# jkulhanek/viewformer

Hardware: NVIDIA H100
Metric: novel views/sec (128x128, 9-ctx) (higher is better)
Workload: dtype f32 encoder (bit-exact codes) + bf16 transformer/decoder

## Files before the change

### include/vf_b200.h

```cpp
#ifndef VF_B200_H
#define VF_B200_H

#include <stdint.h>

#ifdef __cplusplus
extern "C" {
#endif

typedef void* vf_stream_t;

enum { VF_F32 = 0, VF_BF16 = 1, VF_F16X2 = 2  };
enum { VF_ACT_NONE = 0, VF_ACT_GELU_ERF = 1 };
enum { VF_BIAS_NONE = 0, VF_BIAS_N = 1, VF_BIAS_M = 2 };
enum { VF_OK = 0, VF_ERR_ARG = -1, VF_ERR_CUDA = -2, VF_ERR_UNSUPPORTED = -3 };

const char* vf_last_error(void);
int vf_version(void);
int vf_sizeof_simt_gemm(void);
int vf_sizeof_tc_gemm(void);
int vf_device_check(void);

int vf_u8_to_unit_f32(const uint8_t* in, float* out, int64_t rows, int64_t row_len, int64_t in_row_stride, vf_stream_t s);
int vf_unit_f32_to_u8(const float* in, uint8_t* out, int64_t n, vf_stream_t s);
int vf_nchw_to_nhwc_f32(const float* in, float* out, int N, int C, int H, int W, vf_stream_t s);
// ... 17 lines not shown
                 void* y, int y_dtype, vf_stream_t s);

typedef struct {
    const void* A; int a_dtype; int conv;
    int N, H, W, Cin;
    int OH, OW, KH, KW, stride, pad_t, pad_l, upsample2x;
    int64_t a_sm, a_sk;
    const void* B; int b_dtype; int64_t b_sk, b_sn;
    int M, Ncols, K;
    int batch1, batch2;
    int64_t a_sb1, a_sb2, b_sb1, b_sb2, c_sb1, c_sb2;
    float alpha; const float* bias; int bias_mode; int act;
    const float* residual;
    float* C_f32; void* C_bf16;
    int64_t ldc;
} vf_simt_gemm_t;
int vf_simt_gemm(const vf_simt_gemm_t* p, vf_stream_t s);

typedef struct {
    int conv;
    int ab_dtype;
    const void* A; const void* B;
    int M, Ncols, K; int batch1, batch2;
    int64_t lda, ldb;
    int64_t a_sb1, a_sb2, b_sb1, b_sb2;
    int N, H, W, Ctot, Cin, OH, OW, ntaps;
    int tap_dy[9], tap_dx[9], tap_coff[9];
    int causal_block, causal_skip_n;
    float alpha; const float* bias; int bias_mode; int act; const float* residual;
    float* C_f32; void* C_bf16; int64_t ldc, c_sb1, c_sb2;
    double* gn_sums; int gn_groups; int gn_rows_per_img;
    const float* norm_mean_rstd; const float* norm_gamma; const float* norm_beta; int norm_groups; int norm_swish;
    int64_t exact_lo_a, exact_lo_b;
} vf_tc_gemm_t;
int vf_tc_gemm(const vf_tc_gemm_t* p, vf_stream_t s);

int vf_attn_block_causal(const void* qk, const void* vt, int B, int S, int H, int d, int block, void* out, vf_stream_t s);
int vf_attn_block_causal_tail(const void* qk_bf16, const void* vt_bf16, int B, int S, int H, int d, int block, int first_query,
                              void* out_bf16, vf_stream_t s);
int vf_attn_block_causal_decode(const void* qk_bf16, const void* vt_bf16, int B, int S, int H, int d, int block, int first_query,
                                int skip_view, void* out_bf16, vf_stream_t s);
int vf_attn_block_multiend(const void* qk_bf16, const void* vt_bf16, int B, int S, int n_streams, int stream, int H, int d, int block,
                           void* out_bf16, vf_stream_t s);
int vf_attn_multiend_train(const void* qk_bf16, const void* vt_bf16, int B, int S, int n_streams, int stream, int H, int d, int block,
                           float rate, uint64_t seed, float* lse, float* out_f32, void* out_bf16, vf_stream_t s);
int vf_attn_multiend_bwd(const void* qk_bf16, const void* vt_bf16, const void* dout_bf16, const float* out, const float* lse, int B, int S,
                         int n_streams, int H, int d, int block, float rate, uint64_t seed, float* dvqk, vf_stream_t s);

int vf_conv_wgrad(const float* x, const float* dy, int N, int H, int W, int Cin, int OH, int OW, int Cout, int KH, int KW, int stride,
                  int pad_t, int pad_l, int upsample2x, int64_t so_k, int64_t so_n, float* dw, vf_stream_t s);
int vf_col_sums(const float* x, int64_t rows, int C, float* out, vf_stream_t s);
int vf_groupnorm_bwd(const float* x, const float* dout, const float* mean_rstd, const float* gamma, const float* beta, int N, int HW,
                     int C, int groups, int swish, const float* add, double* gsums, float* dgamma, float* dbeta, float* dx, void* dx_bf16,
                     vf_stream_t s);
int vf_softmax_bwd_rows(const float* P, const float* dP, int64_t rows, int cols, float* dS, vf_stream_t s);
int vf_l1_grad(const float* x, const float* y, int64_t n, float scale, float* dy, double* loss_sum, vf_stream_t s);
int vf_lincomb3(float a, const float* x, float b, const float* y, float c, const float* z, int64_t n, float* out, vf_stream_t s);
int vf_pad_transpose_split(const float* x_nhwc, int N, int H, int W, int C, int pitch, int copies, int64_t margin, int64_t L, void* out_f16,
                           vf_stream_t s);
int vf_sum_splits(const float* partial, int groups, int splits, int64_t n, int accumulate, float* out, vf_stream_t s);
typedef struct { const float* w_kn; void* fw_bf16; void* bw_bf16; int64_t cin, cout; } vf_conv_weights_bf16_t;
int vf_pad_transpose_bf16(const float* x_nhwc, int N, int H, int W, int C, int upsample2x, int pitch, int copies, int64_t margin, int64_t L,
                          const float* mean_rstd, const float* gamma, const float* beta, int groups, int swish, void* out_bf16, vf_stream_t s);
int vf_conv_weights_bf16(const vf_conv_weights_bf16_t* table, int n, vf_stream_t s);
int vf_sumpool2x2(const float* x, int N, int H, int W, int C, float* y, vf_stream_t s);
int vf_adam(float* p, const float* g, float* m, float* v, int64_t n, float lr, float beta1, float beta2, float eps, int step,
// ... 61 lines not shown
```

### viewformer_b200/_lib.py

```python
import ctypes as C
import os

import torch

HERE = os.path.dirname(os.path.abspath(__file__))
LIB_PATH = os.environ.get("VF_B200_LIB") or os.path.join(HERE, "libvf_b200.so")

F32, BF16, F16X2 = 0, 1, 2
ACT_NONE, ACT_GELU = 0, 1
BIAS_NONE, BIAS_N, BIAS_M = 0, 1, 2

EXPORTS = [
    "vf_last_error", "vf_version", "vf_sizeof_simt_gemm", "vf_sizeof_tc_gemm", "vf_device_check", "vf_u8_to_unit_f32", "vf_unit_f32_to_u8",
    "vf_nchw_to_nhwc_f32", "vf_nhwc_to_nchw_f32", "vf_groupnorm_stats", "vf_groupnorm_apply", "vf_layernorm",
    "vf_simt_gemm", "vf_tc_gemm", "vf_vq_lookup", "vf_gather_rows", "vf_vq_ema_stats", "vf_vq_ema_update", "vf_vq_commit_grad",
    "vf_vq_prepare_codebook", "vf_migt_embed", "vf_softmax_rows", "vf_argmax_rows", "vf_pose_postprocess",
    "vf_cameras_prepare", "vf_cameras_from_relative",
    "vf_conv3x3_small_cin", "vf_conv3x3_small_cout", "vf_groupnorm_finalize", "vf_split_f16x2", "vf_attn_block_causal", "vf_attn_block_causal_tail", "vf_attn_block_causal_decode", "vf_attn_block_multiend",
    "vf_vq_split3", "vf_vq_select", "vf_cross_entropy_rows", "vf_pose_loss_rows", "vf_row_mean",
    "vf_vq_prepare_codebook_f16", "vf_vq_lookup_fused", "vf_resize_u8", "vf_image_pair_sums", "vf_ssim_u8", "vf_ssim_u8_k",
    "vf_conv_wgrad", "vf_pad_transpose_split", "vf_pad_transpose_bf16", "vf_conv_weights_bf16", "vf_sum_splits", "vf_col_sums", "vf_groupnorm_bwd", "vf_softmax_bwd_rows", "vf_l1_grad", "vf_lincomb3", "vf_sumpool2x2", "vf_adam",
    "vf_layernorm_bwd", "vf_gelu_fwd", "vf_gelu_bwd", "vf_migt_embed_bwd", "vf_cross_entropy_grad", "vf_pose_loss_grad", "vf_adamw_keras", "vf_sumsq", "vf_dropout",
    "vf_attn_multiend_train", "vf_attn_multiend_bwd", "vf_to_bf16", "vf_dense_weights_bf16",
]
# ... 1 lines not shown

class SimtGemm(C.Structure):
    _fields_ = [
        ("A", C.c_void_p), ("a_dtype", C.c_int), ("conv", C.c_int),
        ("N", C.c_int), ("H", C.c_int), ("W", C.c_int), ("Cin", C.c_int),
        ("OH", C.c_int), ("OW", C.c_int), ("KH", C.c_int), ("KW", C.c_int), ("stride", C.c_int),
        ("pad_t", C.c_int), ("pad_l", C.c_int), ("upsample2x", C.c_int),
        ("a_sm", C.c_int64), ("a_sk", C.c_int64),
        ("B", C.c_void_p), ("b_dtype", C.c_int), ("b_sk", C.c_int64), ("b_sn", C.c_int64),
        ("M", C.c_int), ("Ncols", C.c_int), ("K", C.c_int), ("batch1", C.c_int), ("batch2", C.c_int),
        ("a_sb1", C.c_int64), ("a_sb2", C.c_int64), ("b_sb1", C.c_int64), ("b_sb2", C.c_int64),
        ("c_sb1", C.c_int64), ("c_sb2", C.c_int64),
        ("alpha", C.c_float), ("bias", C.c_void_p), ("bias_mode", C.c_int), ("act", C.c_int),
        ("residual", C.c_void_p), ("C_f32", C.c_void_p), ("C_bf16", C.c_void_p), ("ldc", C.c_int64),
    ]


class TcGemm(C.Structure):
    _fields_ = [
        ("conv", C.c_int), ("ab_dtype", C.c_int), ("A", C.c_void_p), ("B", C.c_void_p),
        ("M", C.c_int), ("Ncols", C.c_int), ("K", C.c_int), ("batch1", C.c_int), ("batch2", C.c_int),
        ("lda", C.c_int64), ("ldb", C.c_int64),
        ("a_sb1", C.c_int64), ("a_sb2", C.c_int64), ("b_sb1", C.c_int64), ("b_sb2", C.c_int64),
        ("N", C.c_int), ("H", C.c_int), ("W", C.c_int), ("Ctot", C.c_int), ("Cin", C.c_int),
        ("OH", C.c_int), ("OW", C.c_int), ("ntaps", C.c_int),
        ("tap_dy", C.c_int * 9), ("tap_dx", C.c_int * 9), ("tap_coff", C.c_int * 9),
        ("causal_block", C.c_int), ("causal_skip_n", C.c_int),
        ("alpha", C.c_float), ("bias", C.c_void_p), ("bias_mode", C.c_int), ("act", C.c_int),
        ("residual", C.c_void_p), ("C_f32", C.c_void_p), ("C_bf16", C.c_void_p),
        ("ldc", C.c_int64), ("c_sb1", C.c_int64), ("c_sb2", C.c_int64),
        ("gn_sums", C.c_void_p), ("gn_groups", C.c_int), ("gn_rows_per_img", C.c_int),
        ("norm_mean_rstd", C.c_void_p), ("norm_gamma", C.c_void_p), ("norm_beta", C.c_void_p),
        ("norm_groups", C.c_int), ("norm_swish", C.c_int),
        ("exact_lo_a", C.c_int64), ("exact_lo_b", C.c_int64),
    ]


_lib = None
_device_ok = []


class LibraryError(RuntimeError):
    pass


def load(require_device=False):
    global _lib
    if _lib is None:
        if not os.path.exists(LIB_PATH):
            raise LibraryError(f"{LIB_PATH} not found — run `python -m viewformer_b200.build` (no CPU/PyTorch fallback exists)")
        lib = C.CDLL(LIB_PATH)
        lib.vf_last_error.restype = C.c_char_p
        for name in EXPORTS:
            if not hasattr(lib, name):
                raise LibraryError(f"{LIB_PATH} does not export {name}")
            if name != "vf_last_error":
                getattr(lib, name).restype = C.c_int
        if lib.vf_sizeof_simt_gemm() != C.sizeof(SimtGemm) or lib.vf_sizeof_tc_gemm() != C.sizeof(TcGemm):
            raise LibraryError("parameter struct layout mismatch between _lib.py and include/vf_b200.h")
        _lib = lib
    if require_device and not _device_ok:
        if not torch.cuda.is_available():
            raise LibraryError("viewformer_b200 needs a CUDA device (sm_90a); no CPU fallback exists")
        rc = _lib.vf_device_check()
        if rc != 0:
            raise LibraryError(_lib.vf_last_error().decode())
        _device_ok.append(True)
# ... 312 lines not shown

def conv3x3_small_cout(x, w_kn, bias):
    lib = load(True)
    _dev(x)
    n, h, w, cin = x.shape
    cout = w_kn.shape[1]
    y = torch.empty((n, h, w, cout), dtype=torch.float32, device=x.device)
    _check(lib.vf_conv3x3_small_cout(_p(x), _dt(x), _p(w_kn), _p(bias), n, h, w, cin, cout, _p(y), _stream()))
    return y


def conv_norm_fusable(x, cout):
    n, h, w, c = x.shape
    return x.dtype == torch.bfloat16 and c % 64 == 0 and cout % 128 == 0 and h >= 32 and w >= 8 and n * h * w * cout < 2 ** 31


def gn_mean_rstd(x, groups=32, eps=1e-6):
    lib = load(True)
    n, h, w, c = x.shape
    stats = torch.empty((n, groups, 2), dtype=torch.float32, device=x.device)
    fused = getattr(x, "_gn_sums", None)
    if fused is not None and fused[1] == groups:
        _check(lib.vf_groupnorm_finalize(_p(fused[0]), n * groups, C.c_double(float(h * w * (c // groups))), C.c_float(eps),
                                         _p(stats), _stream()))
    else:
        if x.dtype != torch.float32:
            raise LibraryError("gn_mean_rstd: a bf16 input needs fused statistics from its producer")
        sums = torch.empty((n, groups, 2), dtype=torch.float64, device=x.device)
        _check(lib.vf_groupnorm_stats(_p(x), n, h * w, c, groups, C.c_float(eps), _p(sums), _p(stats), _stream()))
    return stats


def tc_conv(x, w_nk, bias, *, taps=TAPS_3x3, coffs=None, cin=None, out_hw=None, residual=None, out=None,
            out_dtype=torch.float32, out2=None, gn_groups=0, norm=None):
    lib = load(True)
    _dev(x)
    n, h, w, ctot = x.shape
    split = 2 if x.dtype == torch.float16 else 1
    cin = ctot // split if cin is None else cin
    cout = w_nk.shape[0]
    oh, ow = (h, w) if out_hw is None else out_hw
    if out is None:
        out = torch.empty((n, oh, ow, cout), dtype=out_dtype, device=x.device)
    p = TcGemm()
    p.conv, p.ab_dtype = 1, _dt(x)
    assert w_nk.dtype == x.dtype and w_nk.shape[1] == len(taps) * cin * split
    p.A, p.B = x.data_ptr(), w_nk.data_ptr()
    p.Ncols = cout
    p.N, p.H, p.W, p.Ctot, p.Cin, p.OH, p.OW, p.ntaps = n, h, w, ctot, cin, oh, ow, len(taps)
    for i, (dy, dx) in enumerate(taps):
        p.tap_dy[i], p.tap_dx[i] = dy, dx
        p.tap_coff[i] = 0 if coffs is None else coffs[i]
    p.alpha = 1.0
    p.bias, p.bias_mode = (bias.data_ptr(), BIAS_N) if bias is not None else (None, BIAS_NONE)
    p.act = ACT_NONE
    p.residual = residual.data_ptr() if residual is not None else None
    for o in (out, out2):
        if o is None:
            continue
        if o.dtype == torch.float32:
            p.C_f32 = o.data_ptr()
        else:
            p.C_bf16 = o.data_ptr()
    p.ldc = cout
    sums = None
    if gn_groups and gn_fusable(cout, gn_groups, n * oh * ow, oh * ow, cout):
        sums = torch.empty((n, gn_groups, 2), dtype=torch.float64, device=out.device)
        p.gn_sums, p.gn_groups = sums.data_ptr(), gn_groups
    if norm is not None:
        mr, gamma, beta, ngroups, swish = norm
        _dev(mr, torch.float32); _dev(gamma, torch.float32); _dev(beta, torch.float32)
        p.norm_mean_rstd, p.norm_gamma, p.norm_beta = mr.data_ptr(), gamma.data_ptr(), beta.data_ptr()
        p.norm_groups, p.norm_swish = ngroups, int(swish)
    _check(lib.vf_tc_gemm(C.byref(p), _stream()))
    if sums is not None:
        out._gn_sums = (sums, gn_groups)
    return out


def vq_prepare_codebook(emb_dk):
    lib = load(True)
    _dev(emb_dk, torch.float32)
    d, k = emb_dk.shape
    et = torch.empty((k, d), dtype=torch.float32, device=emb_dk.device)
    esq = torch.empty((k,), dtype=torch.float32, device=emb_dk.device)
    _check(lib.vf_vq_prepare_codebook(_p(emb_dk), d, k, _p(et), _p(esq), _stream()))
    return et, esq


def vq_lookup(z_rows, et, esq, want_quant=True, want_diff=True):
    lib = load(True)
    _dev(z_rows, torch.float32)
    m, d = z_rows.shape
    k = et.shape[0]
    idx = torch.empty((m,), dtype=torch.int64, device=z_rows.device)
    quant = torch.empty((m, d), dtype=torch.float32, device=z_rows.device) if want_quant else None
    dsum = torch.zeros((1,), dtype=torch.float64, device=z_rows.device) if want_diff else None
    _check(lib.vf_vq_lookup(_p(z_rows), _p(et), _p(esq), C.c_int64(m), d, k, _p(idx), _p(quant), _p(dsum), _stream()))
    return idx, quant, dsum


def split_f16x2(x_rows):
    lib = load(True)
    _dev(x_rows, torch.float32)
    rows, c = x_rows.shape
    out = torch.empty((rows, 2 * c), dtype=torch.float16, device=x_rows.device)
# ... 550 lines not shown
```

### viewformer_b200/csrc/vf_common.cuh

```cuda
#pragma once
#include <cuda_runtime.h>
#include <cuda_bf16.h>
#include <stdint.h>
#include <stdio.h>
#include <string.h>
#include "../../include/vf_b200.h"

void vf_set_error(const char* fmt, ...);

struct vf_per_device_flag {
    static constexpr int kMaxDevices = 64;
    bool done[kMaxDevices] = {};
    bool& current() {
        int d = 0;
        if (cudaGetDevice(&d) != cudaSuccess || d < 0 || d >= kMaxDevices) d = 0;
        return done[d];
    }
};

#define VF_CHECK_ARG(cond, ...)                                  \
    do {                                                         \
        if (!(cond)) {                                           \
            vf_set_error(__VA_ARGS__);                           \
            return VF_ERR_ARG;                                   \
        }                                                        \
    } while (0)

#define VF_CHECK_LAUNCH(name)                                                        \
    do {                                                                             \
        cudaError_t e__ = cudaGetLastError();                                        \
        if (e__ != cudaSuccess) {                                                    \
            vf_set_error("%s: launch failed: %s", name, cudaGetErrorString(e__));    \
            return VF_ERR_CUDA;                                                      \
        }                                                                            \
    } while (0)

static inline cudaStream_t vf_s(vf_stream_t s) { return reinterpret_cast<cudaStream_t>(s); }

__device__ __forceinline__ float vf_gelu_erf(float x) {
    return 0.5f * x * (1.0f + erff(x * 0.70710678118654752440f));
}
__device__ __forceinline__ float vf_swish(float x) { return x / (1.0f + expf(-x)); }

__device__ __forceinline__ uint32_t mix32(uint64_t k) {
    k ^= k >> 33; k *= 0xff51afd7ed558ccdULL; k ^= k >> 33; k *= 0xc4ceb9fe1a85ec53ULL; k ^= k >> 33;
    return (uint32_t)k;
}
__host__ __device__ __forceinline__ uint32_t vf_drop_threshold(float rate) { return (uint32_t)fminf(rate * 4294967296.0f, 4294967295.0f); }
__device__ __forceinline__ bool vf_drop_keep(unsigned long long seed, unsigned long long i, uint32_t thr) {
    return mix32(seed * 0x9E3779B97F4A7C15ULL + i) >= thr;
}

__device__ __forceinline__ float warp_sum(float v) {
#pragma unroll
    for (int o = 16; o > 0; o >>= 1) v += __shfl_xor_sync(0xffffffffu, v, o);
    return v;
}
__device__ __forceinline__ float warp_max(float v) {
#pragma unroll
    for (int o = 16; o > 0; o >>= 1) v = fmaxf(v, __shfl_xor_sync(0xffffffffu, v, o));
    return v;
}
```

### viewformer_b200/csrc/vf_norm.cu

```cuda
#include "vf_common.cuh"
#include <cuda_fp16.h>

namespace {

struct f16x2_t { __half h; };
template <typename T> struct out_traits { static constexpr bool fast = false, split = false; };
template <> struct out_traits<__nv_bfloat16> { static constexpr bool fast = true, split = false; };
template <> struct out_traits<f16x2_t> { static constexpr bool fast = false, split = true; };

__global__ void __launch_bounds__(256) gn_stats_kernel(const float* __restrict__ x, int HW, int C, int groups,
                                                       int pix_per_block, double* __restrict__ stats) {
    extern __shared__ double sh[];
    const int n = blockIdx.y;
    const int quads = C >> 2;
    const int lanes = 256 / quads;
    const int cq = threadIdx.x % quads;
    const int pl = threadIdx.x / quads;
    for (int i = threadIdx.x; i < groups * 2; i += 256) sh[i] = 0.0;
    __syncthreads();
    const int p0 = blockIdx.x * pix_per_block;
    const int p1 = min(HW, p0 + pix_per_block);
    float s[4] = {0.f, 0.f, 0.f, 0.f}, ss[4] = {0.f, 0.f, 0.f, 0.f};
    if (pl < lanes) {
        const float4* base = reinterpret_cast<const float4*>(x + (int64_t)n * HW * C) + cq;
// ... 43 lines not shown

template <typename OutT>
__device__ __forceinline__ void store4(OutT* p, float a, float b, float c, float d);
template <>
__device__ __forceinline__ void store4<float>(float* p, float a, float b, float c, float d) {
    *reinterpret_cast<float4*>(p) = make_float4(a, b, c, d);
}
template <>
__device__ __forceinline__ void store4<__nv_bfloat16>(__nv_bfloat16* p, float a, float b, float c, float d) {
    __nv_bfloat162 lo = __floats2bfloat162_rn(a, b), hi = __floats2bfloat162_rn(c, d);
    uint2 u;
    u.x = *reinterpret_cast<uint32_t*>(&lo);
    u.y = *reinterpret_cast<uint32_t*>(&hi);
    *reinterpret_cast<uint2*>(p) = u;
}

template <typename InT>
__device__ __forceinline__ float4 load4(const InT* p);
template <>
__device__ __forceinline__ float4 load4<float>(const float* p) {
    return __ldg(reinterpret_cast<const float4*>(p));
}
template <>
__device__ __forceinline__ float4 load4<__nv_bfloat16>(const __nv_bfloat16* p) {
    const uint2 u = __ldg(reinterpret_cast<const uint2*>(p));
    return make_float4(__uint_as_float(u.x << 16), __uint_as_float(u.x & 0xffff0000u), __uint_as_float(u.y << 16),
                       __uint_as_float(u.y & 0xffff0000u));
}

__device__ __forceinline__ void store4_split(f16x2_t* p, int64_t lo_off, float a, float b, float c, float d) {
    const float v[4] = {a, b, c, d};
    __half hi[4], lo[4];
#pragma unroll
    for (int j = 0; j < 4; ++j) {
        hi[j] = __float2half_rn(v[j]);
        lo[j] = __float2half_rn((v[j] - __half2float(hi[j])) * 2048.0f);
    }
    uint2 uh, ul;
    uh.x = (uint32_t)__half_as_ushort(hi[0]) | ((uint32_t)__half_as_ushort(hi[1]) << 16);
    uh.y = (uint32_t)__half_as_ushort(hi[2]) | ((uint32_t)__half_as_ushort(hi[3]) << 16);
    ul.x = (uint32_t)__half_as_ushort(lo[0]) | ((uint32_t)__half_as_ushort(lo[1]) << 16);
    ul.y = (uint32_t)__half_as_ushort(lo[2]) | ((uint32_t)__half_as_ushort(lo[3]) << 16);
    *reinterpret_cast<uint2*>(p) = uh;
    *reinterpret_cast<uint2*>(p + lo_off) = ul;
}

template <typename OutT>
__device__ __forceinline__ float gn_swish(float v) {
    if constexpr (out_traits<OutT>::fast) return __fdividef(v, 1.0f + __expf(-v));
    else return vf_swish(v);
}

template <typename InT, typename OutT, int kLayout>
__global__ void __launch_bounds__(256) gn_apply_kernel(const InT* __restrict__ x, const float* __restrict__ mr,
                                                       const float* __restrict__ gamma, const float* __restrict__ beta, int H, int W,
                                                       int C, int groups, int normalize, int swish, int pix_per_block,
                                                       OutT* __restrict__ y) {
    const int quads = C >> 2;
    const int lanes = 256 / quads;
    const int cq = threadIdx.x % quads, pl = threadIdx.x / quads;
    const int n = blockIdx.y, HW = H * W;
    float mu[4] = {0.f, 0.f, 0.f, 0.f}, rs[4] = {1.f, 1.f, 1.f, 1.f}, ga[4] = {1.f, 1.f, 1.f, 1.f}, be[4] = {0.f, 0.f, 0.f, 0.f};
    if (normalize) {
        const int cpg = C / groups;
        const float4 g4 = __ldg(reinterpret_cast<const float4*>(gamma) + cq);
        const float4 b4 = __ldg(reinterpret_cast<const float4*>(beta) + cq);
        ga[0] = g4.x; ga[1] = g4.y; ga[2] = g4.z; ga[3] = g4.w;
        be[0] = b4.x; be[1] = b4.y; be[2] = b4.z; be[3] = b4.w;
#pragma unroll
        for (int j = 0; j < 4; ++j) {
            const float2 m = __ldg(reinterpret_cast<const float2*>(mr) + (int64_t)n * groups + (cq * 4 + j) / cpg);
            mu[j] = m.x;
            rs[j] = m.y;
        }
    }
    float sc[4], sh[4];
#pragma unroll
    for (int j = 0; j < 4; ++j) { sc[j] = rs[j] * ga[j]; sh[j] = be[j] - mu[j] * sc[j]; }

    auto body = [&](float4 v, int p) {
        float e[4] = {v.x, v.y, v.z, v.w};
#pragma unroll
        for (int j = 0; j < 4; ++j) {
            if (normalize) {
                if constexpr (out_traits<OutT>::fast) e[j] = fmaf(e[j], sc[j], sh[j]);
                else e[j] = (e[j] - mu[j]) * rs[j] * ga[j] + be[j];
            }
            if (swish) e[j] = gn_swish<OutT>(e[j]);
        }
        if constexpr (out_traits<OutT>::split) {
            if constexpr (kLayout == 0) {
                store4_split(y + ((int64_t)n * HW + p) * (2 * C) + cq * 4, C, e[0], e[1], e[2], e[3]);
            } else if constexpr (kLayout == 2) {
                const int yy = p / W, xx = p - yy * W;
                const int64_t o = (((int64_t)n * (H >> 1) + (yy >> 1)) * (W >> 1) + (xx >> 1)) * (8 * (int64_t)C) + ((yy & 1) * 2 + (xx & 1)) * C + cq * 4;
                store4_split(y + o, 4 * (int64_t)C, e[0], e[1], e[2], e[3]);
            } else {
                const int yy = p / W, xx = p - yy * W;
                const int64_t W2 = 2 * (int64_t)W, C2 = 2 * (int64_t)C;
                const int64_t o = (((int64_t)n * 2 * H + 2 * yy) * W2 + 2 * xx) * C2 + cq * 4;
                store4_split(y + o, C, e[0], e[1], e[2], e[3]);
                store4_split(y + o + C2, C, e[0], e[1], e[2], e[3]);
                store4_split(y + o + W2 * C2, C, e[0], e[1], e[2], e[3]);
                store4_split(y + o + W2 * C2 + C2, C, e[0], e[1], e[2], e[3]);
            }
        } else if constexpr (kLayout == 0) {
            store4<OutT>(y + ((int64_t)n * HW + p) * C + cq * 4, e[0], e[1], e[2], e[3]);
        } else if constexpr (kLayout == 2) {
            const int yy = p / W, xx = p - yy * W;
            const int64_t o = ((((int64_t)n * (H >> 1) + (yy >> 1)) * (W >> 1) + (xx >> 1)) * 4 + ((yy & 1) * 2 + (xx & 1))) * C + cq * 4;
            store4<OutT>(y + o, e[0], e[1], e[2], e[3]);
        } else {
            const int yy = p / W, xx = p - yy * W;
            const int64_t W2 = 2 * (int64_t)W;
            const int64_t o = (((int64_t)n * 2 * H + 2 * yy) * W2 + 2 * xx) * C + cq * 4;
            store4<OutT>(y + o, e[0], e[1], e[2], e[3]);
            store4<OutT>(y + o + C, e[0], e[1], e[2], e[3]);
            store4<OutT>(y + o + W2 * C, e[0], e[1], e[2], e[3]);
            store4<OutT>(y + o + W2 * C + C, e[0], e[1], e[2], e[3]);
// ... 184 lines not shown
```

### viewformer_b200/csrc/vf_tc_gemm.cu

```cuda
#include "vf_wgmma.cuh"
#include <stdlib.h>

namespace {
using namespace vftc;

constexpr int BLOCK_M = 128;
constexpr int ROW_BYTES = 128;
constexpr int A_STAGE_BYTES = BLOCK_M * ROW_BYTES;
constexpr int NUM_EPI_WARPS = 8;
constexpr int NUM_MMA_THREADS = 32 * NUM_EPI_WARPS;
constexpr int NUM_THREADS = NUM_MMA_THREADS + 128;

struct TcParams {
    CUtensorMap tmA, tmB;
    int conv;
    int M, Ncols;
    int num_k_blocks;
    int batch2;
    int tiles_m, tiles_n, total_tiles;
    int a_bm1, a_bm2, b_bm1, b_bm2;
    int TW, TH, TN, tiles_x, tiles_y, OH, OW, Nimg, cin_blocks, bk_elems;
    int tap_dy[9], tap_dx[9], tap_coff[9];
    int gemm_koff;
    int causal_block, causal_skip_n;
    float alpha;
    const float* bias;
    int bias_mode, act;
    const float* residual;
    float* C_f32;
    __nv_bfloat16* C_bf16;
    long long ldc, c_sb1, c_sb2;
    int vec_ok;
    int halo;
    double* gn_sums;
    int gn_groups, gn_cpg, gn_rows_per_img;
    int exact;
    int exact_kc;
    int exact_clog;
    int exact_kpp;
    int exact_lo_b;
    const float2* norm_mr;
    const float* norm_gamma;
    const float* norm_beta;
    int norm_groups, norm_cpg, norm_swish;
};

constexpr float EXACT_LO_SCALE = 1.0f / 2048.0f;

struct TileInfo {
    int m0, n0, b1, b2, img0, oy0, ox0, nkb;
    bool skip;
};

__device__ __forceinline__ TileInfo decode_tile(const TcParams& p, int t, int block_n) {
    TileInfo ti;
    const int n_tile = t % p.tiles_n;
    const int r = t / p.tiles_n;
    const int m_tile = r % p.tiles_m;
    const int bz = r / p.tiles_m;
    ti.b1 = bz / p.batch2;
    ti.b2 = bz % p.batch2;
    ti.m0 = m_tile * BLOCK_M;
    ti.n0 = n_tile * block_n;
    ti.nkb = p.num_k_blocks;
    ti.skip = false;
    if (p.causal_block > 0) {
        const int lim = ((ti.m0 + BLOCK_M - 1) / p.causal_block + 1) * p.causal_block;
        if (p.causal_skip_n) {
            ti.skip = ti.n0 >= lim;
        } else {
            const int kb = (lim + p.bk_elems - 1) / p.bk_elems;
            if (kb < ti.nkb) ti.nkb = kb;
        }
    }
    ti.img0 = ti.oy0 = ti.ox0 = 0;
    if (p.conv) {
        const int tx = m_tile % p.tiles_x;
// ... 289 lines not shown
                prev_halo = this_halo;
                if (kExact && p.halo) {
                    if (++stage == NGH) { stage = 0; phase ^= 1; }
                    if (++cb == p.cin_blocks) { cb = 0; if (++tap == 9) { tap = 0; ++j; } }
                } else if (p.halo) {
                    if (++stage == NGH) { stage = 0; phase ^= 1; }
                    if (++tap == 9) { tap = 0; if (++ab == 2) { ab = 0; aphase ^= 1; } }
                } else {
                    if (++stage == NG) { stage = 0; phase ^= 1; }
                }
                if (kExact && ++in_chunk == p.exact_kc) {
                    in_chunk = 0;
                    wgmma_wait<0>();
                    reg_fence(acc);
                    const float sc = (ck < nsmall ? EXACT_LO_SCALE : 1.0f) * p.alpha;
                    if (ck == 0) {
#pragma unroll
                        for (int i = 0; i < NACC; ++i) csum[i] = acc[i] * sc;
                    } else {
#pragma unroll
                        for (int i = 0; i < NACC; ++i) csum[i] = fmaf(acc[i], sc, csum[i]);
                    }
                    ++ck;
                    fresh = true;
                }
            }
            wgmma_wait<0>();
            reg_fence(acc);
            retire_prev();
        };
        if constexpr (kExact) k_loop();

        const int row = quarter * 32 + lane;
        long long my_off;
        int my_ok, gm;
        if (p.conv) {
            const int lx = row % p.TW;
            const int q = row / p.TW;
            const int ly = q % p.TH;
            const int ln = q / p.TH;
            const int img = ti.img0 + ln, oy = ti.oy0 + ly, ox = ti.ox0 + lx;
            my_ok = (img < p.Nimg) && (oy < p.OH) && (ox < p.OW);
            gm = (img * p.OH + oy) * p.OW + ox;
            my_off = (long long)gm * p.ldc;
        } else {
            gm = ti.m0 + row;
            my_ok = gm < p.M;
            my_off = (long long)ti.b1 * p.c_sb1 + (long long)ti.b2 * p.c_sb2 + (long long)gm * p.ldc;
        }
        const float bias_m = (p.bias_mode == VF_BIAS_M && my_ok) ? __ldg(p.bias + gm) : 0.f;

        constexpr int VPR = HALF_N / 4;
        constexpr int RPI = 32 / VPR;
        constexpr int ITERS = 32 / RPI;
        const int r_sub = lane / VPR;
        const int c_ln = (lane % VPR) * 4;
        const int n_ln = ti.n0 + col_half * HALF_N + c_ln;
        const bool fast = p.vec_ok && (ti.n0 + kBlockN <= p.Ncols);
        auto residual_at = [&](int i) {
            const int rr = i * RPI + r_sub;
            const int ok = __shfl_sync(0xffffffffu, my_ok, rr);
            const long long off_row = __shfl_sync(0xffffffffu, my_off, rr);
            const long long o = ok ? off_row + n_ln : (long long)n_ln;
            return __ldg(reinterpret_cast<const float4*>(p.residual + o));
        };
        constexpr int RB = kExact ? ITERS / 2 : ITERS;
        float4 resv[RB];
        auto load_residual = [&](int i0) {
            if (fast && p.residual) {
#pragma unroll
                for (int i = 0; i < RB; ++i) resv[i] = residual_at(i0 + i);
            }
        };
        if constexpr (!kExact) load_residual(0);
        float4 bias4 = make_float4(0.f, 0.f, 0.f, 0.f);
        if (fast && p.bias_mode == VF_BIAS_N) bias4 = __ldg(reinterpret_cast<const float4*>(p.bias + n_ln));

        if constexpr (!kExact) k_loop();
        named_sync(1, NUM_MMA_THREADS);
        if constexpr (kExact) to_staging(csum, 1.0f);
        else to_staging(acc, p.alpha);
        named_sync(1, NUM_MMA_THREADS);

        if (fast) {
            float gs = 0.f, gq = 0.f;
#pragma unroll
            for (int i = 0; i < ITERS; ++i) {
                if (kExact && i % RB == 0) load_residual(i);
                const int rr = i * RPI + r_sub;
                const int ok = __shfl_sync(0xffffffffu, my_ok, rr);
                const long long off_row = __shfl_sync(0xffffffffu, my_off, rr);
                const float bm = __shfl_sync(0xffffffffu, bias_m, rr);
                float4 v = *reinterpret_cast<const float4*>(stg + rr * STG_LD + c_ln);
                if (p.bias_mode == VF_BIAS_N) { v.x += bias4.x; v.y += bias4.y; v.z += bias4.z; v.w += bias4.w; }
                else { v.x += bm; v.y += bm; v.z += bm; v.w += bm; }
                if (p.act == VF_ACT_GELU_ERF) { v.x = vf_gelu_erf(v.x); v.y = vf_gelu_erf(v.y); v.z = vf_gelu_erf(v.z); v.w = vf_gelu_erf(v.w); }
                if (p.residual) {
                    const float4 r = resv[i % RB];
                    v.x += r.x; v.y += r.y; v.z += r.z; v.w += r.w;
                }
                if (ok) {
                    gs += (v.x + v.y) + (v.z + v.w);
                    gq += (v.x * v.x + v.y * v.y) + (v.z * v.z + v.w * v.w);
                    const long long off = off_row + n_ln;
                    if (p.C_f32) *reinterpret_cast<float4*>(p.C_f32 + off) = v;
                    if (p.C_bf16) {
                        __nv_bfloat162 lo = __floats2bfloat162_rn(v.x, v.y), hi = __floats2bfloat162_rn(v.z, v.w);
                        uint2 u;
                        u.x = *reinterpret_cast<uint32_t*>(&lo);
                        u.y = *reinterpret_cast<uint32_t*>(&hi);
                        *reinterpret_cast<uint2*>(p.C_bf16 + off) = u;
                    }
                }
            }
            if (p.gn_sums) {
                const unsigned okmask = __ballot_sync(0xffffffffu, my_ok);
#pragma unroll
                for (int o = VPR; o < 32; o <<= 1) {
                    gs += __shfl_xor_sync(0xffffffffu, gs, o);
                    gq += __shfl_xor_sync(0xffffffffu, gq, o);
                }
                const int lpg = p.gn_cpg >> 2;
                for (int o = 1; o < lpg; o <<= 1) {
                    gs += __shfl_xor_sync(0xffffffffu, gs, o);
                    gq += __shfl_xor_sync(0xffffffffu, gq, o);
                }
                const int gm_first = __shfl_sync(0xffffffffu, gm, okmask ? (__ffs(okmask) - 1) : 0);
                if (okmask && r_sub == 0 && (lane % lpg) == 0) {
                    const long long slot = ((long long)(gm_first / p.gn_rows_per_img) * p.gn_groups + n_ln / p.gn_cpg) * 2;
                    atomicAdd(p.gn_sums + slot, (double)gs);
                    atomicAdd(p.gn_sums + slot + 1, (double)gq);
                }
            }
// ... 39 lines not shown
        return VF_ERR_CUDA;
    }
    return VF_OK;
}

template <int kBlockN, int kStages, WgKind kKind>
int launch(const TcParams& prm, dim3 grid, cudaStream_t st) {
    constexpr int smem = tc_smem_bytes<kBlockN, kStages, kKind == F16>();
    static_assert(kStages <= MAX_STAGES, "ring depth");
    static_assert(smem <= 232448, "shared memory budget");
    static vf_per_device_flag configured_pd;
    bool& configured = configured_pd.current();
    if (!configured) {
        cudaError_t e = cudaFuncSetAttribute(tc_gemm_kernel<kBlockN, kStages, kKind>, cudaFuncAttributeMaxDynamicSharedMemorySize, smem);
        if (e != cudaSuccess) { vf_set_error("vf_tc_gemm: cudaFuncSetAttribute: %s", cudaGetErrorString(e)); return VF_ERR_CUDA; }
        configured = true;
    }
    tc_gemm_kernel<kBlockN, kStages, kKind><<<grid, NUM_THREADS, smem, st>>>(prm);
    VF_CHECK_LAUNCH("vf_tc_gemm");
    return VF_OK;
}

template <int kBlockN, int kStages>
int launch_kind(const TcParams& prm, WgKind kind, dim3 grid, cudaStream_t st) {
    if (kind == TF32) return launch<kBlockN, kStages, TF32>(prm, grid, st);
    if (kind == F16) return launch<kBlockN, kStages, F16>(prm, grid, st);
    return launch<kBlockN, kStages, BF16>(prm, grid, st);
}

}

extern "C" int vf_tc_gemm(const vf_tc_gemm_t* q, vf_stream_t s) {
    VF_CHECK_ARG(q && q->A && q->B, "vf_tc_gemm: null operand");
    VF_CHECK_ARG(q->C_f32 || q->C_bf16, "vf_tc_gemm: no output");
    VF_CHECK_ARG(q->ab_dtype == VF_BF16 || q->ab_dtype == VF_F32 || q->ab_dtype == VF_F16X2, "vf_tc_gemm: bad dtype");
    const bool exact = q->ab_dtype == VF_F16X2;
    if (exact) {
        VF_CHECK_ARG(q->C_f32 && !q->C_bf16 && !q->norm_mean_rstd && q->causal_block == 0,
                     "vf_tc_gemm: VF_F16X2 (exact split-fp16) operands need an fp32 output and no causal / fused-norm options");
        if (q->conv) VF_CHECK_ARG(q->Ctot % 2 == 0 && q->alpha == 1.0f, "vf_tc_gemm: exact conv needs [hi | lo] channels and alpha = 1");
        else VF_CHECK_ARG(q->K % 64 == 0 && q->exact_lo_a >= q->K && q->exact_lo_b >= q->K && q->exact_lo_a % 8 == 0 && q->exact_lo_b % 8 == 0,
                          "vf_tc_gemm: exact GEMM needs K %% 64 == 0 and lo-half offsets >= K (K=%d lo_a=%lld lo_b=%lld)", q->K,
                          (long long)q->exact_lo_a, (long long)q->exact_lo_b);
    }
    VF_CHECK_ARG(q->bias_mode == VF_BIAS_NONE || q->bias, "vf_tc_gemm: bias pointer missing");
    VF_CHECK_ARG(!q->norm_mean_rstd || q->conv, "vf_tc_gemm: fused input GroupNorm is a convolution option");
    const bool tf32 = q->ab_dtype == VF_F32;
    const int tm_dtype = tf32 ? VF_F32 : VF_BF16;
    const int es = tf32 ? 4 : 2;
    const int bk = ROW_BYTES / es;

    TcParams prm;
    memset(&prm, 0, sizeof(prm));
    prm.conv = q->conv;
    prm.Ncols = q->Ncols;
    prm.bk_elems = bk;
    prm.alpha = q->alpha;
    prm.bias = q->bias;
    prm.bias_mode = q->bias_mode;
    prm.act = q->act;
    prm.residual = q->residual;
    prm.C_f32 = q->C_f32;
    prm.C_bf16 = reinterpret_cast<__nv_bfloat16*>(q->C_bf16);
    prm.ldc = q->ldc;
    prm.causal_block = q->causal_block;
    prm.causal_skip_n = q->causal_skip_n;

    const int block_n = (q->Ncols > 64) ? 128 : 64;
    const int b_box_rows = block_n;
    dim3 grid;
    int rc;
    if (q->conv) {
// ... 80 lines not shown
        prm.a_bm1 = (q->batch1 > 1 && q->a_sb1 != 0) ? 1 : 0;
        prm.a_bm2 = (q->batch2 > 1 && q->a_sb2 != 0) ? 1 : 0;
        prm.b_bm1 = (q->batch1 > 1 && q->b_sb1 != 0) ? 1 : 0;
        prm.b_bm2 = (q->batch2 > 1 && q->b_sb2 != 0) ? 1 : 0;
        const uint64_t fbA = (uint64_t)q->lda * es * (uint64_t)q->M, fbB = (uint64_t)q->ldb * es * (uint64_t)q->Ncols;
        const uint64_t dimsA[4] = {(uint64_t)((exact ? q->exact_lo_a + q->K : q->K) + max_koff), (uint64_t)q->M, prm.a_bm2 ? (uint64_t)q->batch2 : 1, prm.a_bm1 ? (uint64_t)q->batch1 : 1};
        const uint64_t strA[3] = {(uint64_t)q->lda * es, prm.a_bm2 ? (uint64_t)q->a_sb2 * es : fbA, prm.a_bm1 ? (uint64_t)q->a_sb1 * es : fbA};
        const uint32_t boxA[4] = {(uint32_t)bk, (uint32_t)BLOCK_M, 1, 1};
        if ((rc = make_tmap(&prm.tmA, tm_dtype, q->A, dimsA, strA, boxA)) != VF_OK) return rc;
        const uint64_t dimsB[4] = {(uint64_t)(exact ? q->exact_lo_b + q->K : q->K), (uint64_t)q->Ncols, prm.b_bm2 ? (uint64_t)q->batch2 : 1, prm.b_bm1 ? (uint64_t)q->batch1 : 1};
        const uint64_t strB[3] = {(uint64_t)q->ldb * es, prm.b_bm2 ? (uint64_t)q->b_sb2 * es : fbB, prm.b_bm1 ? (uint64_t)q->b_sb1 * es : fbB};
        const uint32_t boxB[4] = {(uint32_t)bk, (uint32_t)b_box_rows, 1, 1};
        if ((rc = make_tmap(&prm.tmB, tm_dtype, q->B, dimsB, strB, boxB)) != VF_OK) return rc;
        VF_CHECK_ARG(q->causal_block == 0 || (q->causal_block % bk == 0 || bk % q->causal_block == 0), "vf_tc_gemm: causal block");
        grid = dim3((q->M + BLOCK_M - 1) / BLOCK_M, (q->Ncols + block_n - 1) / block_n, q->batch1 * q->batch2);
    }
    prm.tiles_m = (int)grid.x;
    prm.tiles_n = (int)grid.y;
    const long long total = (long long)prm.tiles_m * grid.y * grid.z;
    VF_CHECK_ARG(total > 0 && total < (1ll << 31), "vf_tc_gemm: tile count out of range");
    prm.total_tiles = (int)total;
    static int num_sms = 0;
    if (num_sms == 0) {
        int dev = 0;
        cudaGetDevice(&dev);
        if (cudaDeviceGetAttribute(&num_sms, cudaDevAttrMultiProcessorCount, dev) != cudaSuccess || num_sms <= 0) num_sms = 132;
    }
    const dim3 pgrid((unsigned)(total < num_sms ? total : num_sms), 1, 1);
    {
        auto a16 = [](const void* p) { return (reinterpret_cast<uintptr_t>(p) & 15) == 0; };
        auto a8 = [](const void* p) { return (reinterpret_cast<uintptr_t>(p) & 7) == 0; };
        prm.vec_ok = (q->ldc % 4 == 0) && (q->c_sb1 % 4 == 0) && (q->c_sb2 % 4 == 0) && a16(q->C_f32) && a8(q->C_bf16) && a16(q->residual) &&
                     a16(q->bias);
    }
    if (q->gn_sums) {
        const int C = q->Ncols;
        VF_CHECK_ARG(q->gn_groups > 0 && C % q->gn_groups == 0, "vf_tc_gemm: gn_groups");
        const int cpg = C / q->gn_groups;
        const long long rpi = q->conv ? (long long)q->OH * q->OW : q->gn_rows_per_img;
        const long long rows = q->conv ? (long long)q->N * q->OH * q->OW : (long long)q->M;
        VF_CHECK_ARG(cpg % 4 == 0 && cpg <= 32 && 32 % cpg == 0 && C % block_n == 0 && prm.vec_ok && rpi >= 32 && rpi % 32 == 0 &&
                         rows % rpi == 0 && (q->conv ? (prm.TW * prm.TH) % 32 == 0 : q->batch1 * q->batch2 == 1),
                     "vf_tc_gemm: fused GroupNorm statistics unsupported for this shape (C=%d groups=%d rows/img=%lld)", C, q->gn_groups, rpi);
        prm.gn_sums = q->gn_sums;
        prm.gn_groups = q->gn_groups;
        prm.gn_cpg = cpg;
        prm.gn_rows_per_img = (int)rpi;
        cudaError_t e = cudaMemsetAsync(q->gn_sums, 0, sizeof(double) * 2 * q->gn_groups * (rows / rpi), vf_s(s));
        if (e != cudaSuccess) { vf_set_error("vf_tc_gemm: memset gn_sums: %s", cudaGetErrorString(e)); return VF_ERR_CUDA; }
    }
    cudaStream_t st = vf_s(s);
    const WgKind kind = tf32 ? TF32 : (exact ? F16 : BF16);
    if (block_n == 128) return launch_kind<128, 4>(prm, kind, pgrid, st);
    return launch_kind<64, 6>(prm, kind, pgrid, st);
}
```

### viewformer_b200/vqgan.py

```python
import re
from collections import OrderedDict

import os

import torch

from . import _lib as L
from .config import VQGANConfig, load_config
from .ops import Precision, Linear, gemm_nt, linear

_IGNORE = re.compile(r"(perceptual_loss\..*)|(loss\..*)")


class _Conv3:

    def __init__(self, w, b, prec, device, *, exact=False):
        cout, cin, kh, kw = w.shape
        self.cout, self.cin, self.k = cout, cin, kh
        w = w.to(device=device, dtype=torch.float32)
        self.bias = b.to(device=device, dtype=torch.float32).contiguous()
        self.tc = (not exact) and prec.use_tc and kh == 3 and cin % prec.k_align == 0 and cout % 16 == 0 and cout >= 64
        self.small_cin = kh == 3 and cin == 3 and cout % 16 == 0 and cout <= 128
        self.small_cout = kh == 3 and cin == 128 and cout == 3
        if self.tc and prec.split:
# ... 252 lines not shown
        self._w = w
        self._refresh_codebook()

    def _refresh_codebook(self):
        q = self._w["q"]
        q["et"], q["esq"] = L.vq_prepare_codebook(q["emb"])
        q["et3"] = L.vq_split3(q["et"], True) if self.prec.use_tc else None
        q["eh"] = L.vq_prepare_codebook_f16(q["et"]) if (self.prec.use_tc and L.vq_fused_ok(*q["emb"].shape)) else None
        self._refresh_decode_table()

    def _refresh_decode_table(self):
        q = self._w["q"]
        self._w["pq_table"] = linear(self.exact, q["et"], self._w["post_quant_conv"], torch.float32)

    def _conv(self, cw, x_opd_or_f32, *, residual=None, stride=1, upsample=False, stats=True, out_dtype=torch.float32):
        gn = 32 if stats else 0
        if cw.tc and stride == 2:
            return L.tc_conv(x_opd_or_f32, cw.w_nk, cw.bias, taps=L.TAPS_S2D, coffs=L.s2d_coffs(cw.cin), cin=cw.cin, gn_groups=gn)
        if cw.tc:
            return L.tc_conv(x_opd_or_f32, cw.w_nk, cw.bias, residual=residual, gn_groups=gn, out_dtype=out_dtype)
        assert out_dtype == torch.float32
        if stride == 1 and not upsample and residual is None and x_opd_or_f32.dtype == torch.float32:
            if cw.small_cin:
                return L.conv3x3_small_cin(x_opd_or_f32, cw.w_kn, cw.bias, gn_groups=gn)
            if cw.small_cout:
                return L.conv3x3_small_cout(x_opd_or_f32, cw.w_kn, cw.bias)
        pad = (1, 1) if stride == 1 else (0, 0)
        return L.simt_conv(x_opd_or_f32, cw.w_kn, cw.bias, kh=cw.k, stride=stride, pad=pad if cw.k == 3 else (0, 0),
                           upsample=upsample, residual=residual)

    def _act_dtype(self, cw, prec):
        return prec.opd if cw.tc else torch.float32

    def _resblock(self, rbw, x):
        prec = rbw["prec"]
        bf16 = prec.name == "bf16"
        a = L.groupnorm(x, *rbw["n1"], swish=True, out_dtype=self._act_dtype(rbw["c1"], prec))
        n_, h_, w_, _ = x.shape
        c1 = rbw["c1"]
        edge = torch.bfloat16 if (bf16 and self.bf16_edges and c1.tc and rbw["c2"].tc
                                  and L.gn_fusable(c1.cout, 32, n_ * h_ * w_, h_ * w_, c1.cout)) else torch.float32
        h = self._conv(c1, a, out_dtype=edge)
        if h.dtype == torch.bfloat16 and self.norm_on_load and L.conv_norm_fusable(h, rbw["c2"].cout):
            a, norm2 = h, (L.gn_mean_rstd(h), rbw["n2"][0], rbw["n2"][1], 32, True)
        else:
            a, norm2 = L.groupnorm(h, *rbw["n2"], swish=True, out_dtype=self._act_dtype(rbw["c2"], prec)), None
        if "sc" in rbw:
            n, hh, ww, c = x.shape
            lp = rbw["lprec"]
            xs = x if lp.opd == torch.float32 else L.groupnorm(x, None, None, swish=False, out_dtype=lp.opd, normalize=False)
            res = linear(lp, xs.reshape(n * hh * ww, -1), rbw["sc"], torch.float32).reshape(n, hh, ww, -1)
        else:
            res = x
        if norm2 is not None:
            return L.tc_conv(a, rbw["c2"].w_nk, rbw["c2"].bias, residual=res, gn_groups=32, norm=norm2)
        return self._conv(rbw["c2"], a, residual=res)

    def _attn(self, aw, x):
        prec = aw["prec"]
        if prec.split:
            return self._attn_exact(aw, x)
        n, hh, ww, c = x.shape
        hw = hh * ww
        a = L.groupnorm(x, *aw["norm"], swish=False, out_dtype=prec.opd).reshape(n * hw, c)
        qk = linear(prec, a, aw["qk"], prec.opd)
        vt = torch.empty((n, c, hw), dtype=prec.opd, device=x.device)
        gemm_nt(prec, aw["v"].w, a, vt, M=c, N=hw, K=c, lda=c, ldb=c, ldc=hw, batch=(n, 1), a_bs=(0, 0),
                b_bs=(hw * c, 0), c_bs=(c * hw, 0), bias=aw["v"].b, bias_mode=L.BIAS_M)
        scores = torch.empty((n, hw, hw), dtype=torch.float32, device=x.device)
        gemm_nt(prec, qk, qk, scores, M=hw, N=hw, K=c, lda=2 * c, ldb=2 * c, ldc=hw, batch=(n, 1),
                a_bs=(hw * 2 * c, 0), b_bs=(hw * 2 * c, 0), c_bs=(hw * hw, 0), b_off=c, alpha=float(int(c) ** (-0.5)))
        p = torch.empty((n, hw, hw), dtype=prec.opd, device=x.device)
        L.softmax_rows(scores, p, rows_total=n * hw, rows_per_batch=hw, cols=hw, ld_in=hw, ld_out=hw)
        o = torch.empty((n * hw, c), dtype=prec.opd, device=x.device)
        gemm_nt(prec, p, vt, o, M=hw, N=c, K=hw, lda=hw, ldb=hw, ldc=c, batch=(n, 1), a_bs=(hw * hw, 0),
                b_bs=(c * hw, 0), c_bs=(hw * c, 0))
        out = linear(prec, o, aw["proj"], torch.float32, residual=x.reshape(n * hw, c), gn_rows_per_img=hw)
        out4 = out.reshape(n, hh, ww, c)
        if hasattr(out, "_gn_sums"):
            out4._gn_sums = out._gn_sums
        return out4

    def _attn_exact(self, aw, x):
        prec = aw["prec"]
        n, hh, ww, c = x.shape
        hw = hh * ww
        f32 = torch.float32
        a = L.groupnorm(x, *aw["norm"], swish=False, out_dtype=torch.float16).reshape(n * hw, 2 * c)
        qk = linear(prec, a, aw["qk"], f32)
        qks = L.split_f16x2(qk)
        vt = torch.empty((n, c, hw), dtype=f32, device=x.device)
        gemm_nt(prec, aw["v"].w, a, vt, M=c, N=hw, K=c, lda=2 * c, ldb=2 * c, ldc=hw, batch=(n, 1), a_bs=(0, 0),
                b_bs=(hw * 2 * c, 0), c_bs=(c * hw, 0), bias=aw["v"].b, bias_mode=L.BIAS_M)
        scores = torch.empty((n, hw, hw), dtype=f32, device=x.device)
        gemm_nt(prec, qks, qks, scores, M=hw, N=hw, K=c, lda=4 * c, ldb=4 * c, ldc=hw, batch=(n, 1), a_bs=(hw * 4 * c, 0),
                b_bs=(hw * 4 * c, 0), c_bs=(hw * hw, 0), b_off=c, alpha=float(int(c) ** (-0.5)), lo_a=2 * c, lo_b=2 * c)
        p = torch.empty((n, hw, hw), dtype=f32, device=x.device)
        L.softmax_rows(scores, p, rows_total=n * hw, rows_per_batch=hw, cols=hw, ld_in=hw, ld_out=hw)
        ps = L.split_f16x2(p.reshape(n * hw, hw))
        vts = L.split_f16x2(vt.reshape(n * c, hw))
        o = torch.empty((n * hw, c), dtype=f32, device=x.device)
        gemm_nt(prec, ps, vts, o, M=hw, N=c, K=hw, lda=2 * hw, ldb=2 * hw, ldc=c, batch=(n, 1), a_bs=(hw * 2 * hw, 0),
                b_bs=(c * 2 * hw, 0), c_bs=(hw * c, 0))
        out = linear(prec, L.split_f16x2(o), aw["proj"], f32, residual=x.reshape(n * hw, c), gn_rows_per_img=hw)
        out4 = out.reshape(n, hh, ww, c)
        if hasattr(out, "_gn_sums"):
            out4._gn_sums = out._gn_sums
        return out4

    def _encoder_level(self, lvw, h):
        for i, rbw in enumerate(lvw["blocks"]):
            h = self._resblock(rbw, h)
            if lvw["attns"]:
                h = self._attn(lvw["attns"][i], h)
        if lvw["down"] is not None:
            down = lvw["down"]
            if down.tc and h.shape[1] % 2 == 0 and h.shape[2] % 2 == 0:
                hs = L.groupnorm(h, None, None, swish=False, out_dtype=self.enc_prec.opd, normalize=False, s2d=True)
                h = self._conv(down, hs, stride=2)
            else:
                if down.tc:
                    raise NotImplementedError("odd feature-map size in Downsample on the tensor-core path")
                h = self._conv(down, h, stride=2)
        return h

    def _encoder(self, x):
        e = self._w["enc"]
        n = x.shape[0]
        chunk, nlev = self.encoder_chunk, min(self.encoder_chunk_levels, len(e["levels"]))
        if chunk > 0 and n > chunk:
            parts = []
            for i in range(0, n, chunk):
                h = self._conv(e["conv_in"], x[i:i + chunk])
                for lvw in e["levels"][:nlev]:
                    h = self._encoder_level(lvw, h)
                parts.append(h)
            h = torch.cat(parts, 0)
            if all(hasattr(p, "_gn_sums") for p in parts):
                h._gn_sums = (torch.cat([p._gn_sums[0] for p in parts], 0), parts[0]._gn_sums[1])
            rest = e["levels"][nlev:]
        else:
            h = self._conv(e["conv_in"], x)
            rest = e["levels"]
        for lvw in rest:
# ... 170 lines not shown
```

Baseline: 247.9.

## Fuse space-to-depth split-fp16 output into last resblock conv before downsample

In the exact (split fp16) encoder path, the last resblock's second conv before a downsample now writes its output directly in space-to-depth layout as hi/lo fp16 halves. This replaces a separate groupnorm-based s2d/split pass and the fp32 intermediate round-trip. The GN helpers are rewritten with explicit rounding intrinsics to keep the fused result bit-exact with the standalone path.

```diff
diff --git a/include/vf_b200.h b/include/vf_b200.h
--- a/include/vf_b200.h
+++ b/include/vf_b200.h
@@ -73,6 +73,7 @@
     double* gn_sums; int gn_groups; int gn_rows_per_img;
     const float* norm_mean_rstd; const float* norm_gamma; const float* norm_beta; int norm_groups; int norm_swish;
     int64_t exact_lo_a, exact_lo_b;
+    void* C_s2d_f16x2;
 } vf_tc_gemm_t;
 int vf_tc_gemm(const vf_tc_gemm_t* p, vf_stream_t s);
 
diff --git a/viewformer_b200/_lib.py b/viewformer_b200/_lib.py
--- a/viewformer_b200/_lib.py
+++ b/viewformer_b200/_lib.py
@@ -57,7 +57,7 @@
         ("gn_sums", C.c_void_p), ("gn_groups", C.c_int), ("gn_rows_per_img", C.c_int),
         ("norm_mean_rstd", C.c_void_p), ("norm_gamma", C.c_void_p), ("norm_beta", C.c_void_p),
         ("norm_groups", C.c_int), ("norm_swish", C.c_int),
-        ("exact_lo_a", C.c_int64), ("exact_lo_b", C.c_int64),
+        ("exact_lo_a", C.c_int64), ("exact_lo_b", C.c_int64), ("C_s2d_f16x2", C.c_void_p),
     ]
 
 
@@ -436,7 +436,7 @@
 
 
 def tc_conv(x, w_nk, bias, *, taps=TAPS_3x3, coffs=None, cin=None, out_hw=None, residual=None, out=None,
-            out_dtype=torch.float32, out2=None, gn_groups=0, norm=None):
+            out_dtype=torch.float32, out2=None, gn_groups=0, norm=None, s2d_split=False):
     lib = load(True)
     _dev(x)
     n, h, w, ctot = x.shape
@@ -444,7 +444,10 @@
     cin = ctot // split if cin is None else cin
     cout = w_nk.shape[0]
     oh, ow = (h, w) if out_hw is None else out_hw
-    if out is None:
+    if s2d_split:
+        assert out is None and out2 is None and not gn_groups
+        s2d = torch.empty((n, oh // 2, ow // 2, 8 * cout), dtype=torch.float16, device=x.device)
+    elif out is None:
         out = torch.empty((n, oh, ow, cout), dtype=out_dtype, device=x.device)
     p = TcGemm()
     p.conv, p.ab_dtype = 1, _dt(x)
@@ -476,6 +479,10 @@
         _dev(mr, torch.float32); _dev(gamma, torch.float32); _dev(beta, torch.float32)
         p.norm_mean_rstd, p.norm_gamma, p.norm_beta = mr.data_ptr(), gamma.data_ptr(), beta.data_ptr()
         p.norm_groups, p.norm_swish = ngroups, int(swish)
+    if s2d_split:
+        p.C_s2d_f16x2 = s2d.data_ptr()
+        _check(lib.vf_tc_gemm(C.byref(p), _stream()))
+        return s2d
     _check(lib.vf_tc_gemm(C.byref(p), _stream()))
     if sums is not None:
         out._gn_sums = (sums, gn_groups)
diff --git a/viewformer_b200/csrc/vf_common.cuh b/viewformer_b200/csrc/vf_common.cuh
--- a/viewformer_b200/csrc/vf_common.cuh
+++ b/viewformer_b200/csrc/vf_common.cuh
@@ -1,6 +1,7 @@
 #pragma once
 #include <cuda_runtime.h>
 #include <cuda_bf16.h>
+#include <cuda_fp16.h>
 #include <stdint.h>
 #include <stdio.h>
 #include <string.h>
@@ -42,6 +43,14 @@
 }
 __device__ __forceinline__ float vf_swish(float x) { return x / (1.0f + expf(-x)); }
 
+__device__ __forceinline__ float vf_gn_exact(float e, float mu, float rs, float ga, float be) {
+    return __fmaf_rn(__fmul_rn(__fsub_rn(e, mu), rs), ga, be);
+}
+__device__ __forceinline__ void vf_split_f16(float v, __half& hi, __half& lo) {
+    hi = __float2half_rn(v);
+    lo = __float2half_rn(__fmul_rn(__fsub_rn(v, __half2float(hi)), 2048.0f));
+}
+
 __device__ __forceinline__ uint32_t mix32(uint64_t k) {
     k ^= k >> 33; k *= 0xff51afd7ed558ccdULL; k ^= k >> 33; k *= 0xc4ceb9fe1a85ec53ULL; k ^= k >> 33;
     return (uint32_t)k;
diff --git a/viewformer_b200/csrc/vf_norm.cu b/viewformer_b200/csrc/vf_norm.cu
--- a/viewformer_b200/csrc/vf_norm.cu
+++ b/viewformer_b200/csrc/vf_norm.cu
@@ -99,10 +99,7 @@
     const float v[4] = {a, b, c, d};
     __half hi[4], lo[4];
 #pragma unroll
-    for (int j = 0; j < 4; ++j) {
-        hi[j] = __float2half_rn(v[j]);
-        lo[j] = __float2half_rn((v[j] - __half2float(hi[j])) * 2048.0f);
-    }
+    for (int j = 0; j < 4; ++j) vf_split_f16(v[j], hi[j], lo[j]);
     uint2 uh, ul;
     uh.x = (uint32_t)__half_as_ushort(hi[0]) | ((uint32_t)__half_as_ushort(hi[1]) << 16);
     uh.y = (uint32_t)__half_as_ushort(hi[2]) | ((uint32_t)__half_as_ushort(hi[3]) << 16);
@@ -151,7 +148,7 @@
         for (int j = 0; j < 4; ++j) {
             if (normalize) {
                 if constexpr (out_traits<OutT>::fast) e[j] = fmaf(e[j], sc[j], sh[j]);
-                else e[j] = (e[j] - mu[j]) * rs[j] * ga[j] + be[j];
+                else e[j] = vf_gn_exact(e[j], mu[j], rs[j], ga[j], be[j]);
             }
             if (swish) e[j] = gn_swish<OutT>(e[j]);
         }
diff --git a/viewformer_b200/csrc/vf_tc_gemm.cu b/viewformer_b200/csrc/vf_tc_gemm.cu
--- a/viewformer_b200/csrc/vf_tc_gemm.cu
+++ b/viewformer_b200/csrc/vf_tc_gemm.cu
@@ -43,6 +43,7 @@
     const float* norm_gamma;
     const float* norm_beta;
     int norm_groups, norm_cpg, norm_swish;
+    __half* C_s2d;
 };
 
 constexpr float EXACT_LO_SCALE = 1.0f / 2048.0f;
@@ -398,7 +399,7 @@
         if constexpr (kExact) k_loop();
 
         const int row = quarter * 32 + lane;
-        long long my_off;
+        long long my_off, my_s2d = 0;
         int my_ok, gm;
         if (p.conv) {
             const int lx = row % p.TW;
@@ -409,6 +410,8 @@
             my_ok = (img < p.Nimg) && (oy < p.OH) && (ox < p.OW);
             gm = (img * p.OH + oy) * p.OW + ox;
             my_off = (long long)gm * p.ldc;
+            if constexpr (kExact)
+                my_s2d = ((long long)(img * (p.OH >> 1) + (oy >> 1)) * (p.OW >> 1) + (ox >> 1)) * (8 * p.ldc) + ((oy & 1) * 2 + (ox & 1)) * p.ldc;
         } else {
             gm = ti.m0 + row;
             my_ok = gm < p.M;
@@ -465,6 +468,24 @@
                     const float4 r = resv[i % RB];
                     v.x += r.x; v.y += r.y; v.z += r.z; v.w += r.w;
                 }
+                if constexpr (kExact) {
+                    if (p.C_s2d) {
+                        const long long o2 = __shfl_sync(0xffffffffu, my_s2d, rr) + n_ln;
+                        if (ok) {
+                            const float e[4] = {v.x, v.y, v.z, v.w};
+                            __half hi[4], lo[4];
+#pragma unroll
+                            for (int j = 0; j < 4; ++j) vf_split_f16(e[j], hi[j], lo[j]);
+                            *reinterpret_cast<uint2*>(p.C_s2d + o2) =
+                                make_uint2((uint32_t)__half_as_ushort(hi[0]) | ((uint32_t)__half_as_ushort(hi[1]) << 16),
+                                           (uint32_t)__half_as_ushort(hi[2]) | ((uint32_t)__half_as_ushort(hi[3]) << 16));
+                            *reinterpret_cast<uint2*>(p.C_s2d + o2 + 4 * p.ldc) =
+                                make_uint2((uint32_t)__half_as_ushort(lo[0]) | ((uint32_t)__half_as_ushort(lo[1]) << 16),
+                                           (uint32_t)__half_as_ushort(lo[2]) | ((uint32_t)__half_as_ushort(lo[3]) << 16));
+                        }
+                        continue;
+                    }
+                }
                 if (ok) {
                     gs += (v.x + v.y) + (v.z + v.w);
                     gq += (v.x * v.x + v.y * v.y) + (v.z * v.z + v.w * v.w);
@@ -570,12 +591,13 @@
 
 extern "C" int vf_tc_gemm(const vf_tc_gemm_t* q, vf_stream_t s) {
     VF_CHECK_ARG(q && q->A && q->B, "vf_tc_gemm: null operand");
-    VF_CHECK_ARG(q->C_f32 || q->C_bf16, "vf_tc_gemm: no output");
+    VF_CHECK_ARG(q->C_f32 || q->C_bf16 || q->C_s2d_f16x2, "vf_tc_gemm: no output");
     VF_CHECK_ARG(q->ab_dtype == VF_BF16 || q->ab_dtype == VF_F32 || q->ab_dtype == VF_F16X2, "vf_tc_gemm: bad dtype");
     const bool exact = q->ab_dtype == VF_F16X2;
     if (exact) {
-        VF_CHECK_ARG(q->C_f32 && !q->C_bf16 && !q->norm_mean_rstd && q->causal_block == 0,
-                     "vf_tc_gemm: VF_F16X2 (exact split-fp16) operands need an fp32 output and no causal / fused-norm options");
+        VF_CHECK_ARG(!q->C_f32 != !q->C_s2d_f16x2 && !q->C_bf16 && !q->norm_mean_rstd && q->causal_block == 0,
+                     "vf_tc_gemm: VF_F16X2 (exact split-fp16) operands need one fp32 or split space-to-depth output and no causal / "
+                     "fused-norm options");
         if (q->conv) VF_CHECK_ARG(q->Ctot % 2 == 0 && q->alpha == 1.0f, "vf_tc_gemm: exact conv needs [hi | lo] channels and alpha = 1");
         else VF_CHECK_ARG(q->K % 64 == 0 && q->exact_lo_a >= q->K && q->exact_lo_b >= q->K && q->exact_lo_a % 8 == 0 && q->exact_lo_b % 8 == 0,
                           "vf_tc_gemm: exact GEMM needs K %% 64 == 0 and lo-half offsets >= K (K=%d lo_a=%lld lo_b=%lld)", q->K,
@@ -722,6 +744,14 @@
         auto a8 = [](const void* p) { return (reinterpret_cast<uintptr_t>(p) & 7) == 0; };
         prm.vec_ok = (q->ldc % 4 == 0) && (q->c_sb1 % 4 == 0) && (q->c_sb2 % 4 == 0) && a16(q->C_f32) && a8(q->C_bf16) && a16(q->residual) &&
                      a16(q->bias);
+        if (q->C_s2d_f16x2) {
+            VF_CHECK_ARG(exact && q->conv && q->OH % 2 == 0 && q->OW % 2 == 0 && q->ldc == q->Ncols && q->Ncols % block_n == 0 &&
+                             !q->gn_sums && prm.vec_ok && a8(q->C_s2d_f16x2),
+                         "vf_tc_gemm: the split space-to-depth output needs an exact conv with even OH, OW (%dx%d), ldc = Cout = a "
+                         "multiple of %d, 16-byte aligned bias / residual, an 8-byte aligned output and no GroupNorm statistics",
+                         q->OH, q->OW, block_n);
+            prm.C_s2d = reinterpret_cast<__half*>(q->C_s2d_f16x2);
+        }
     }
     if (q->gn_sums) {
         const int C = q->Ncols;
diff --git a/viewformer_b200/vqgan.py b/viewformer_b200/vqgan.py
--- a/viewformer_b200/vqgan.py
+++ b/viewformer_b200/vqgan.py
@@ -308,7 +308,7 @@
     def _act_dtype(self, cw, prec):
         return prec.opd if cw.tc else torch.float32
 
-    def _resblock(self, rbw, x):
+    def _resblock(self, rbw, x, s2d=False):
         prec = rbw["prec"]
         bf16 = prec.name == "bf16"
         a = L.groupnorm(x, *rbw["n1"], swish=True, out_dtype=self._act_dtype(rbw["c1"], prec))
@@ -330,6 +330,8 @@
             res = x
         if norm2 is not None:
             return L.tc_conv(a, rbw["c2"].w_nk, rbw["c2"].bias, residual=res, gn_groups=32, norm=norm2)
+        if s2d:
+            return L.tc_conv(a, rbw["c2"].w_nk, rbw["c2"].bias, residual=res, s2d_split=True)
         return self._conv(rbw["c2"], a, residual=res)
 
     def _attn(self, aw, x):
@@ -385,7 +387,11 @@
         return out4
 
     def _encoder_level(self, lvw, h):
+        down = lvw["down"]
         for i, rbw in enumerate(lvw["blocks"]):
+            if (i == len(lvw["blocks"]) - 1 and not lvw["attns"] and down is not None and down.tc and rbw["prec"].split
+                    and rbw["c2"].tc and h.shape[1] % 2 == 0 and h.shape[2] % 2 == 0):
+                return self._conv(down, self._resblock(rbw, h, s2d=True), stride=2)
             h = self._resblock(rbw, h)
             if lvw["attns"]:
                 h = self._attn(lvw["attns"][i], h)
```

After: 250.2, median of 6. Within noise of the previous version (+1.0%).
